# RandomMike1280/AlphaZero-Reversi

Measured on AMD Instinct MI355X. Metric: self-play board-steps/sec @ 800 sims/move, 8x8 Reversi, higher is better.
Workload: dtype u64 rules + f32 NN (fp32 as 2-part f16 split on MFMA)

## Files before the change

### alphazero-reversi_amd/csrc/rvz_play.hip

```cpp
#include <hip/hip_runtime.h>
#include <math.h>
#include <stdint.h>
#include <stdio.h>
#include <stdlib.h>

#include <string>
#include <vector>

#include "../../include/rvz.h"
#include "rvz_engine_host.h"
#include "rvz_h2.hip.h"
#include "rvz_host.hip.h"
#include "rvz_play.hip.h"
#include "rvz_search.hip.h"
#include "rvz_trace.h"

using namespace rvz;


__global__ void k_table_bump(unsigned* gen) {
    if (threadIdx.x == 0) atomicAdd(gen, 1u);
}

int table_bump(rvz_engine* e) {
    if (!e->tgen) return RVZ_OK;
    hipLaunchKernelGGL(k_table_bump, dim3(1), dim3(64), 0, e->stream, e->tgen);
    RVZ_HIP(hipGetLastError(), e);
    return RVZ_OK;
}

void table_free(rvz_engine* e) {
    for (void* p : {(void*)e->tab, (void*)e->tclaim, (void*)e->tgen})
        if (p) (void)hipFree(p);
    e->tab = nullptr;
    e->tclaim = nullptr;
    e->tgen = nullptr;
    e->tslots = 0;
    e->tab_blob = nullptr;
}

extern "C" {

int rvz_play_gate(rvz_engine* e, double fraction, double timeout_us, double late_us) {
    if (!e || !(fraction <= 1.0) || !(timeout_us >= 0.0) || !(late_us >= 0.0) ||
        timeout_us > 1e6 || late_us > 1e6) {
        if (e) e->err = "rvz_play_gate: fraction <= 1 (< 0: the default), 0 <= us <= 1e6";
        return RVZ_EINVAL;
    }
    e->gate_frac = fraction;
    e->gate_us = timeout_us;
    e->gate_late_us = late_us;
    return RVZ_OK;
}

int rvz_play_table(rvz_engine* e, int64_t slots, int32_t max_discs) {
    if (!e) return RVZ_EINVAL;
    if (slots != 0 && (slots < 1024 || (slots & (slots - 1)) != 0 || slots > (1ll << 30) ||
                       max_discs < 4)) {
        e->err = "rvz_play_table: slots a power of two in [1024, 2^30] (or 0), max_discs >= 4";
        return RVZ_EINVAL;
    }
    RVZ_HIP(hipStreamSynchronize(e->stream), e);
    if (slots == e->tslots && slots != 0) {
        e->tmaxd = max_discs;
        return table_bump(e);
    }
    table_free(e);
    if (slots == 0) return RVZ_OK;
    const size_t stride = e->BS == 8 ? TabGeo<8>::STRIDE : TabGeo<6>::STRIDE;
    if (hipMalloc(reinterpret_cast<void**>(&e->tab), (size_t)slots * stride * 8) != hipSuccess ||
        hipMalloc(reinterpret_cast<void**>(&e->tclaim), (size_t)slots * 4) != hipSuccess ||
        hipMalloc(reinterpret_cast<void**>(&e->tgen), 4) != hipSuccess) {
        table_free(e);
        e->err = "hipMalloc failed (rvz_play_table)";
        return RVZ_ENOMEM;
    }
    hipError_t st = hipMemset(e->tab, 0, (size_t)slots * stride * 8);
    if (st == hipSuccess) st = hipMemset(e->tclaim, 0, (size_t)slots * 4);
    if (st == hipSuccess) st = hipMemsetD32(e->tgen, 1u, 1);
    if (st == hipSuccess) st = hipDeviceSynchronize();
    if (st != hipSuccess) {
        table_free(e);
        e->err = std::string("rvz_play_table init: ") + hipGetErrorString(st);
        return RVZ_EHIP;
    }
    e->tslots = slots;
    e->tmaxd = max_discs;
    return RVZ_OK;
}

#ifdef RVZ_WALK_STATS
int rvz_play_walk_read(int32_t n_games, uint64_t* out) {
    const int n = n_games < WALK_STATS_MAX ? n_games : WALK_STATS_MAX;
    std::vector<unsigned long long> a, b;
    if (take_rows(g_wtime, n, a) != RVZ_OK || take_rows(g_ftime, n, b) != RVZ_OK) return RVZ_EHIP;
    for (int i = 0; i < n; ++i) {
        for (int k = 0; k < 5; ++k) out[(size_t)i * 9 + k] = a[(size_t)i * 5 + k];
        for (int k = 0; k < 4; ++k) out[(size_t)i * 9 + 5 + k] = b[(size_t)i * 4 + k];
    }
    return RVZ_OK;
}
#endif

struct PlayScratch {
    int64_t q_next, q_done, gate, queue, x, need, work, logits, value, total;
};
static PlayScratch play_scratch(int64_t G, int NSQ, int NPOL) {
    const auto al4 = [](int64_t n) { return (n + 3) / 4 * 4; };
    int64_t at = 0;
    const auto take = [&](int64_t words) { const int64_t o = at; at += al4(words); return o; };
    PlayScratch s;
    s.q_next = take(4);
    s.q_done = take(2 * al4(G));
    s.gate = take(8 * 32);
    s.queue = at;
    s.x = take(G * 3 * NSQ);
    s.need = take(G);
    s.work = take(G * 192);
    s.logits = take(G * NPOL);
    s.value = take(G);
    s.total = at;
    return s;
}
int64_t rvz_play_scratch_size(const rvz_engine* e) {
    if (!e) return RVZ_EINVAL;
    return play_scratch(e->v.G, e->NSQ, e->NPOL).total;
}

#ifndef RVZ_PLAY_GROUP
#define RVZ_PLAY_GROUP 4
#endif
#ifndef RVZ_PLAY_GATE_FRAC
#define RVZ_PLAY_GATE_FRAC 0.8
#endif
#ifndef RVZ_PLAY_GATE_US
#define RVZ_PLAY_GATE_US 400.0
#endif
#ifndef RVZ_PLAY_GATE_LATE_US
#define RVZ_PLAY_GATE_LATE_US 200.0
#endif
extern "C++" {
template <class T>
static int play_launch(rvz_engine* e, const View& v, const PlayArgs& pa) {
    constexpr int F = T::F, BS = T::BS;
    int cus = 0;
    if (hipDeviceGetAttribute(&cus, hipDeviceAttributeMultiprocessorCount, e->cfg.device) !=
            hipSuccess || cus <= 0)
        cus = 256;
    PlayArgs a = pa;
    const int slots = cus * T::OCC;
    dim3 grid;
    if (a.q_next) {
        if (a.gpw <= 0) a.gpw = RVZ_PLAY_GROUP;
        if (a.gpw > play_gpw_max<F, BS>()) a.gpw = play_gpw_max<F, BS>();
        a.n_groups = (v.G + a.gpw - 1) / a.gpw;
        grid = dim3(a.n_groups < slots ? a.n_groups : slots);
        RVZ_HIP(fill32_async(a.q_next, 0u, (size_t)play_scratch(v.G, e->NSQ, e->NPOL).queue,
                             e->stream), e);
    } else {
        if (a.gpw <= 0) a.gpw = (v.G + slots - 1) / slots;
        if (a.gpw > play_gpw_max<F, BS>()) a.gpw = play_gpw_max<F, BS>();
        a.n_groups = (v.G + a.gpw - 1) / a.gpw;
        grid = dim3(a.n_groups);
    }
    PlayCtx ctx;
    ctx.v = v;
    ctx.a = a;
    hipLaunchKernelGGL((k_play<T::F, T::NB, T::CTW, T::PTW, T::BS, T::OCC>), grid, dim3(256), 0,
                       e->stream, ctx);
    return launch_check(e, "k_play");
}
}

#ifdef RVZ_PLAY_TIMING
int rvz_play_timing_read(uint64_t* host, int n) {
    if (hipMemcpyFromSymbol(host, HIP_SYMBOL(g_play_t), (size_t)n * PLAY_T_SLOTS * 8) != hipSuccess)
        return RVZ_EHIP;
    if (hipMemcpyFromSymbol(host + (size_t)n * PLAY_T_SLOTS, HIP_SYMBOL(g_pass_t),
                            (size_t)n * 6 * 8) != hipSuccess)
        return RVZ_EHIP;
    std::vector<unsigned long long> z((size_t)16384 * PLAY_T_SLOTS, 0ull);
    if (hipMemcpyToSymbol(HIP_SYMBOL(g_pass_t), z.data(), (size_t)16384 * 6 * 8) != hipSuccess)
        return RVZ_EHIP;
    return hipMemcpyToSymbol(HIP_SYMBOL(g_play_t), z.data(), z.size() * 8) == hipSuccess
               ? RVZ_OK : RVZ_EHIP;
}
#endif

struct PlayGate {
    unsigned frac, t, late;
};
static PlayGate play_gate_setting(const rvz_engine* e, bool queue) {
    double frac = e->gate_frac, us = e->gate_us, late = e->gate_late_us;
    if (frac < 0.0) {
        frac = RVZ_PLAY_GATE_FRAC;
        us = RVZ_PLAY_GATE_US;
        late = RVZ_PLAY_GATE_LATE_US;
    }
    if (const char* gs = getenv("RVZ_PLAY_GATE")) {
        double f = 0.0, u = 0.0, l = 0.0;
        const int n = sscanf(gs, "%lf,%lf,%lf", &f, &u, &l);
        frac = n >= 2 ? f : 0.0;
        us = u;
        late = n >= 3 ? l : 0.0;
    }
    PlayGate g;
    g.frac = (queue && frac > 0.0 && us > 0.0) ? (unsigned)(fmin(frac, 1.0) * 65536.0 + 0.5) : 0u;
    g.t = (unsigned)(us * 100.0);
    g.late = late > 0.0 ? (unsigned)(late * 100.0) : 0u;
    return g;
}

int rvz_play(rvz_engine* e, const rvz_play_args* a) {
    const Range trace_range("rvz.play (fused search + h2 evaluator)");
    if (!e || !a) return RVZ_EINVAL;
    if (!a->params || !a->blob || !a->scratch || !a->seeds || !a->plies_done || !a->out_idx ||
        !a->out_p || (a->reset && !a->games_done) || a->plies < 1 || a->blocks < 0 ||
        !h2_tile_ok(e->BS, a->filters) || a->games_per_workgroup < -PLAY_GPW_MAX ||
        e->cfg.leaf_dtype != RVZ_LEAF_F32) {
        e->err = "rvz_play: invalid arguments";
        return RVZ_EINVAL;
    }
    if ((((uintptr_t)a->params | (uintptr_t)a->blob | (uintptr_t)a->scratch) & 15) != 0) {
        e->err = "rvz_play: params, blob and scratch must be 16-byte aligned";
        return RVZ_EINVAL;
    }
    if (in_search(e, "rvz_play")) return RVZ_EINVAL;
    View v = e->v;
    v.live = nullptr;
    v.row_of = nullptr;
    v.live_total = nullptr;
    v.stats = nullptr;
    if ((a->rec_black || a->rec_white || a->rec_side || a->rec_p) &&
        !(a->rec_black && a->rec_white && a->rec_side && a->rec_p)) {
        e->err = "rvz_play: rec_black, rec_white, rec_side and rec_p go together";
        return RVZ_EINVAL;
    }
    PlayArgs pa;
    pa.prm = a->params;
    pa.L = make_layout(a->filters, a->blocks, e->BS);
    pa.blob = a->blob;
    pa.n_blocks = a->blocks;
    pa.ovf = a->ovf;
    const PlayScratch sc = play_scratch(v.G, e->NSQ, e->NPOL);
    const bool queue = a->games_per_workgroup <= 0;
    pa.q_next = queue ? reinterpret_cast<unsigned*>(a->scratch + sc.q_next) : nullptr;
    pa.q_done = queue ? reinterpret_cast<unsigned long long*>(a->scratch + sc.q_done) : nullptr;
    pa.gate = queue ? reinterpret_cast<unsigned long long*>(a->scratch + sc.gate) : nullptr;
    pa.x = a->scratch + sc.x;
    pa.need = reinterpret_cast<int32_t*>(a->scratch + sc.need);
    pa.work = a->scratch + sc.work;
    pa.logits = a->scratch + sc.logits;
    pa.value = a->scratch + sc.value;
    pa.n_groups = 0;
    pa.gpw = queue ? -a->games_per_workgroup : a->games_per_workgroup;
    const PlayGate gate = play_gate_setting(e, queue);
    pa.gate_frac = gate.frac;
    pa.gate_t = gate.t;
    pa.gate_late = gate.late;
    pa.spin_limit = 1u << 26;
    if (const char* sl = getenv("RVZ_PLAY_SPIN_LIMIT")) pa.spin_limit = (unsigned)strtoul(sl, nullptr, 10);
    pa.single_pass = 1;
    if (const char* sp = getenv("RVZ_PLAY_SINGLE_PASS")) pa.single_pass = atoi(sp) != 0;
    pa.S = e->cfg.num_simulations;
    pa.B = e->cfg.batch_size;
    pa.skip_last = a->skip_last_eval && pa.S > pa.B ? 1 : 0;
    pa.skip_forced = a->skip_forced_roots && pa.skip_last ? 1 : 0;
    pa.plies = a->plies;
    pa.budget = a->ply_budget;
    pa.temperature = a->temperature;
    pa.reset = a->reset ? 1 : 0;
    pa.seeds = a->seeds;
    pa.stride = a->seed_stride;
    pa.ply_ctr = a->plies_done;
    pa.done = a->games_done;
    pa.out_idx = a->out_idx;
    pa.out_p = a->out_p;
    pa.hist = a->hist;
    pa.rows = reinterpret_cast<unsigned long long*>(a->rows_evaluated);
    pa.unread = reinterpret_cast<unsigned long long*>(a->rows_unread);
    pa.roots_unread = reinterpret_cast<unsigned long long*>(a->roots_unread);
    pa.tstats = reinterpret_cast<unsigned long long*>(a->table_stats);
    pa.rec_black = a->rec_black;
    pa.rec_white = a->rec_white;
    pa.rec_side = a->rec_side;
    pa.rec_p = a->rec_p;
    pa.tab = nullptr;
    pa.tclaim = nullptr;
    pa.tgen = nullptr;
    pa.tmask = 0;
    pa.tmaxd = 0;
    if (e->tab) {
        if (e->tab_blob != a->blob) {
            if (e->tab_blob) {
                hipStreamCaptureStatus cs = hipStreamCaptureStatusNone;
                if (hipStreamIsCapturing(e->stream, &cs) == hipSuccess &&
                    cs != hipStreamCaptureStatusNone) {
                    e->err = "rvz_play: another weight blob than the table's while the stream is "
                             "capturing (play once eagerly with this evaluator before capturing)";
                    return RVZ_EINVAL;
                }
                const int r = table_bump(e);
                if (r != RVZ_OK) return r;
            }
            e->tab_blob = a->blob;
        }
        pa.tab = e->tab;
        pa.tclaim = e->tclaim;
        pa.tgen = e->tgen;
        pa.tmask = (unsigned)(e->tslots - 1);
        pa.tmaxd = e->tmaxd;
    }
    e->searching = 0;
    int r = RVZ_EINVAL;
    h2_tile(e->BS, a->filters, [&](auto t) { r = play_launch<decltype(t)>(e, v, pa); });
    return r;
}

}
```

### alphazero-reversi_amd/csrc/rvz_play.hip.h

```cpp
#pragma once
#include <hip/hip_runtime.h>
#include <stdint.h>

#include "rvz_h2.hip.h"
#include "rvz_resnet_common.hip.h"
#include "rvz_search.hip.h"

namespace rvz {
namespace {

struct PlayArgs {
    const float* prm;
    Layout L;
    const uint16_t* blob;
    int n_blocks;
    float* x;
    int32_t* need;
    float* work;
    float* logits;
    float* value;
    float* ovf;
    int gpw, plies, skip_last, reset, S, B;
    double temperature;
    int64_t* seeds;
    int64_t stride;
    int64_t* ply_ctr;
    int64_t* done;
    int32_t* out_idx;
    double* out_p;
    int32_t* hist;
    unsigned long long* rows;
    const int32_t* budget;
    unsigned spin_limit;
    int single_pass;
    unsigned long long* tab;
    unsigned* tclaim;
    const unsigned* tgen;
    unsigned tmask;
    int tmaxd;
    unsigned long long* tstats;
    unsigned long long* unread;
    uint64_t* rec_black;
    uint64_t* rec_white;
    int32_t* rec_side;
    double* rec_p;
    unsigned* q_next;
    unsigned long long* q_done;
    int n_groups;
    unsigned long long* gate;
    unsigned gate_frac;
    unsigned gate_t;
    unsigned gate_late;
    int skip_forced;
    unsigned long long* roots_unread;
};
constexpr int PLAY_GPW_MAX = 64;
template <int F, int BS>
__host__ __device__ constexpr bool play_heads_lds() { return F == 64 && BS == 8; }
template <int F, int BS>
__host__ __device__ constexpr int play_gpw_max() {
    return play_heads_lds<F, BS>() ? 8 : PLAY_GPW_MAX;
}
enum : int { PF_QUEUED = 1, PF_READY = 2, PF_DONE = 4, PF_EVAL = 8, PF_HELD = 16 };
constexpr int32_t ERR_SCHED = 16;

template <int BS>
struct TabGeo {
    static constexpr int NSQ = Geo<BS>::NSQ;
    static constexpr int NG = NSQ + 8;
    static constexpr int STRIDE = (NG + 7) / 8 * 8;
};
constexpr int TAB_PROBES = 8;

__device__ __forceinline__ uint64_t tab_mix(uint64_t z) {
    z ^= z >> 30;
    z *= 0xbf58476d1ce4e5b9ull;
    z ^= z >> 27;
    z *= 0x94d049bb133111ebull;
    return z ^ (z >> 31);
}
__device__ __forceinline__ uint64_t tab_hash(uint64_t P, uint64_t O, uint64_t V) {
    return tab_mix(P ^ tab_mix(O ^ tab_mix(V + 0x9e3779b97f4a7c15ull)));
}
template <int NSQ>
__device__ __forceinline__ uint32_t tab_key_word(int idx, uint64_t P, uint64_t O, uint64_t V) {
    const int k = idx - (NSQ + 2);
    const uint64_t w = k < 2 ? P : (k < 4 ? O : V);
    return (k & 1) ? (uint32_t)(w >> 32) : (uint32_t)w;
}

template <int BS>
__device__ __forceinline__ int tab_read(const unsigned long long* __restrict__ tab, uint32_t sl,
                                         uint32_t gen, uint64_t P, uint64_t O, uint64_t V,
                                         int lane, uint64_t& x0, uint64_t& x1) {
    using T = TabGeo<BS>;
    constexpr int NSQ = T::NSQ, NG = T::NG;
    const unsigned long long* e = tab + (size_t)sl * T::STRIDE;
    x0 = 0;
    x1 = 0;
    if (lane < NG) x0 = __hip_atomic_load(e + lane, __ATOMIC_RELAXED, __HIP_MEMORY_SCOPE_AGENT);
    if (NG > 64 && lane < NG - 64)
        x1 = __hip_atomic_load(e + 64 + lane, __ATOMIC_RELAXED, __HIP_MEMORY_SCOPE_AGENT);
    bool stale = false, other = false;
    if (lane < NG) {
        stale |= (uint32_t)(x0 >> 32) != gen;
        if (lane >= NSQ + 2) other |= (uint32_t)x0 != tab_key_word<NSQ>(lane, P, O, V);
    }
    if (NG > 64 && lane < NG - 64) {
        stale |= (uint32_t)(x1 >> 32) != gen;
        if (64 + lane >= NSQ + 2) other |= (uint32_t)x1 != tab_key_word<NSQ>(64 + lane, P, O, V);
    }
    if (__ballot(stale) != 0ull) return 0;
    return __ballot(other) != 0ull ? 1 : 2;
}

template <int BS, int IDX>
__device__ __forceinline__ uint32_t tab_datum(uint64_t x0, uint64_t x1) {
    if constexpr (IDX < 64) return (uint32_t)__builtin_amdgcn_readlane((int)(uint32_t)x0, IDX);
    else return (uint32_t)__builtin_amdgcn_readlane((int)(uint32_t)x1, IDX - 64);
}

template <int BS>
__device__ __forceinline__ bool tab_lookup(const PlayArgs& a, uint32_t gen, uint64_t P,
                                           uint64_t O, uint64_t V, int lane, int g) {
    constexpr int NSQ = Geo<BS>::NSQ, NPOL = Geo<BS>::NPOL;
    const uint64_t h = tab_hash(P, O, V);
    for (int i = 0; i < TAB_PROBES; ++i) {
        const uint32_t sl = (uint32_t)(h + i) & a.tmask;
        uint64_t x0, x1;
        const int r = tab_read<BS>(a.tab, sl, gen, P, O, V, lane, x0, x1);
        if (r == 0) return false;
        if (r == 1) continue;
        float* row = a.logits + (size_t)g * NPOL;
        if (lane < NSQ) row[lane] = __uint_as_float((uint32_t)x0);
        if (lane == 0) {
            row[NSQ] = __uint_as_float(tab_datum<BS, NSQ>(x0, x1));
            a.value[g] = __uint_as_float(tab_datum<BS, NSQ + 1>(x0, x1));
        }
        return true;
    }
    return false;
}

template <int BS>
__device__ __forceinline__ int tab_insert(const PlayArgs& a, uint32_t gen, uint64_t P, uint64_t O,
                                          uint64_t V, int lane, int g) {
    using T = TabGeo<BS>;
    constexpr int NSQ = T::NSQ, NPOL = Geo<BS>::NPOL, NG = T::NG;
    const uint64_t h = tab_hash(P, O, V);
    for (int i = 0; i < TAB_PROBES; ++i) {
        const uint32_t sl = (uint32_t)(h + i) & a.tmask;
        uint32_t c = 0;
        if (lane == 0) c = __hip_atomic_load(a.tclaim + sl, __ATOMIC_RELAXED, __HIP_MEMORY_SCOPE_AGENT);
        c = (uint32_t)__builtin_amdgcn_readfirstlane((int)c);
        if (c == gen) {
            uint64_t x0, x1;
            if (tab_read<BS>(a.tab, sl, gen, P, O, V, lane, x0, x1) == 2) return 0;
            continue;
        }
        uint32_t won = 0;
        if (lane == 0) {
            uint32_t expect = c;
            won = __hip_atomic_compare_exchange_strong(a.tclaim + sl, &expect, gen,
                                                       __ATOMIC_RELAXED, __ATOMIC_RELAXED,
                                                       __HIP_MEMORY_SCOPE_AGENT) ? 1u : 0u;
        }
        if (!__builtin_amdgcn_readfirstlane((int)won)) continue;
        const float* row = a.logits + (size_t)g * NPOL;
        const float val = a.value[g];
        unsigned long long* e = a.tab + (size_t)sl * T::STRIDE;
        const unsigned long long tag = (unsigned long long)gen << 32;
        if (lane < NG) {
            const uint32_t d = lane < NPOL ? __float_as_uint(row[lane])
                               : lane == NSQ + 1 ? __float_as_uint(val)
                                                 : tab_key_word<NSQ>(lane, P, O, V);
            __hip_atomic_store(e + lane, tag | d, __ATOMIC_RELAXED, __HIP_MEMORY_SCOPE_AGENT);
        }
        if (NG > 64 && lane < NG - 64) {
            const int idx = 64 + lane;
            const uint32_t d = idx < NPOL ? __float_as_uint(row[idx])
                               : idx == NSQ + 1 ? __float_as_uint(val)
                                                : tab_key_word<NSQ>(idx, P, O, V);
            __hip_atomic_store(e + idx, tag | d, __ATOMIC_RELAXED, __HIP_MEMORY_SCOPE_AGENT);
        }
        return 1;
    }
    return 0;
}

__device__ __forceinline__ void gate_open(unsigned long long* w, unsigned r) {
    unsigned long long v = __hip_atomic_load(w, __ATOMIC_RELAXED, __HIP_MEMORY_SCOPE_AGENT);
    while ((unsigned)(v >> 32) == r) {
        if (__hip_atomic_compare_exchange_strong(w, &v, (unsigned long long)(r + 1u) << 32,
                                                 __ATOMIC_RELAXED, __ATOMIC_RELAXED,
                                                 __HIP_MEMORY_SCOPE_AGENT)) {
            __hip_atomic_store(w + 1, __builtin_amdgcn_s_memrealtime(), __ATOMIC_RELAXED,
                               __HIP_MEMORY_SCOPE_AGENT);
            return;
        }
    }
}
__device__ __forceinline__ unsigned long long* gate_line(unsigned long long* gate) {
    const unsigned x = (unsigned)__builtin_amdgcn_s_getreg((31 << 11) | 20) & 7u;
    return gate + 16 * x;
}
__device__ __forceinline__ void gate_running(unsigned long long* gate, long long d) {
    __hip_atomic_fetch_add(gate_line(gate) + 2, (unsigned long long)d, __ATOMIC_RELAXED,
                           __HIP_MEMORY_SCOPE_AGENT);
}
__device__ __forceinline__ void play_gate(unsigned long long* gate, unsigned frac, unsigned t,
                                          unsigned late) {
    unsigned long long* w = gate_line(gate);
    if (late) {
        const unsigned long long t_open =
            __hip_atomic_load(w + 1, __ATOMIC_RELAXED, __HIP_MEMORY_SCOPE_AGENT);
        if (t_open && __builtin_amdgcn_s_memrealtime() - t_open < late) return;
    }
    const unsigned long long running =
        __hip_atomic_load(w + 2, __ATOMIC_RELAXED, __HIP_MEMORY_SCOPE_AGENT);
    if (running < 4) return;
    const unsigned k = max(1u, (unsigned)((running * frac) >> 16));
    const unsigned long long old =
        __hip_atomic_fetch_add(w, 1ull, __ATOMIC_RELAXED, __HIP_MEMORY_SCOPE_AGENT);
    const unsigned r = (unsigned)(old >> 32);
    if ((unsigned)old + 1u >= k) {
        gate_open(w, r);
        return;
    }
    const unsigned long long t0 = __builtin_amdgcn_s_memrealtime();
    for (;;) {
        __builtin_amdgcn_s_sleep(2);
        const unsigned long long v = __hip_atomic_load(w, __ATOMIC_RELAXED, __HIP_MEMORY_SCOPE_AGENT);
        if ((unsigned)(v >> 32) != r) return;
        if (__builtin_amdgcn_s_memrealtime() - t0 > t) {
            gate_open(w, r);
            return;
        }
    }
}

struct PlayCtx {
    View v;
    PlayArgs a;
};
__device__ __forceinline__ int opaque_tid() {
    int t = threadIdx.x;
    asm volatile("" : "+v"(t));
    return t;
}
__device__ __forceinline__ const PlayCtx& play_ctx() {
    const __attribute__((address_space(4))) char* p =
        (const __attribute__((address_space(4))) char*)__builtin_amdgcn_kernarg_segment_ptr();
    asm volatile("" : "+s"(p));
    return *(const PlayCtx*)p;
}

#ifdef RVZ_PLAY_TIMING
constexpr int PLAY_T_SLOTS = 14;
__device__ unsigned long long g_play_t[16384][PLAY_T_SLOTS];
#define PT_NOW(t) const unsigned long long t = __builtin_amdgcn_s_memtime()
#define PT_ADD(i, v) if (tid == 0 && blockIdx.x < 16384) g_play_t[blockIdx.x][i] += (v)
#else
#define PT_NOW(t)
#define PT_ADD(i, v)
#endif

template <int F, int NBOARD, int CTW, int PTW, int BS, int OCC>
__global__ __launch_bounds__(256) __attribute__((amdgpu_waves_per_eu(OCC, OCC)))
void k_play(PlayCtx ctx0) {
    (void)ctx0;
    using WT = WaveTilesH<F, CTW, PTW>;
    constexpr bool ILV = RVZ_H2_ILV && NBOARD == 2 && BS == 8 && PTW == 4 && WT::CG == 2;
    using GH = GeoH<NBOARD, BS, 64 * CTW * H2_TM / F, ILV>;
    using C = CfgH<F, GH::NPIX>;
    constexpr int NPOL = Geo<BS>::NPOL;
    constexpr bool HLDS = play_heads_lds<F, BS>();
    constexpr int GMAX = play_gpw_max<F, BS>();
    constexpr bool PLAY_SINGLE = F == 64 && NBOARD == 2 && BS == 8 && (PTW & 1) == 0 && HLDS;
    constexpr int HROW = heads_in_floats(BS) / 16;
    constexpr int SP_BYTES = WPB * (NPOL + 7) * 8;
    static_assert(heads_in_floats(BS) * 4 <= C::RMAX, "heads rows fit");
    static_assert(SP_BYTES + WPB * 624 * 4 <= C::RMAX, "act / reset scratch fits");
    __shared__ __attribute__((aligned(16))) char smem[C::BYTES];
    __shared__ int st_k[GMAX];
    __shared__ int st_f[GMAX];
    __shared__ int st_p[GMAX];
    __shared__ uint64_t st_bits[GMAX * 3];
    __shared__ uint64_t q_bits[(GMAX + NBOARD) * 3];
    __shared__ __attribute__((aligned(16))) float hin[HLDS ? GMAX * HROW : 4];
    __shared__ int q_rows[GMAX + 16];
    __shared__ int s_nq;
    __shared__ float vpart[4][16];
    __shared__ int s_task[2];
    __shared__ unsigned s_tgen;
    const int tid = threadIdx.x;
    const int wave = __builtin_amdgcn_readfirstlane(tid >> 6);
    int E, G, gpw, queue, task_plies;
    {
        const PlayCtx& c = play_ctx();
        E = c.v.E;
        G = c.v.G;
        gpw = c.a.gpw;
        queue = c.a.q_next != nullptr;
        task_plies = queue ? 1 : c.a.plies;
    }
    bool ovf = false;
    __shared__ unsigned s_cnt[5];
    if (tid < 5) s_cnt[tid] = 0u;
    if (tid == 0) {
        const PlayArgs& a = play_ctx().a;
        s_tgen = a.tab ? __hip_atomic_load(a.tgen, __ATOMIC_RELAXED, __HIP_MEMORY_SCOPE_AGENT) : 0u;
    }
    double* sp = reinterpret_cast<double*>(smem) + wave * (NPOL + 7);
    uint32_t* key = reinterpret_cast<uint32_t*>(smem + SP_BYTES) + wave * 624;
    if constexpr (F >= 128 && BS == 8) {
        const PlayArgs& a = play_ctx().a;
        if (tid == 0 && a.gate_frac > 0) gate_running(a.gate, 1);
    }
    PT_NOW(t_start);
    for (int task_i = 0;; ++task_i) {
        int gi, ply0;
        if (!queue) {
            if (task_i > 0) break;
            gi = blockIdx.x;
            ply0 = 0;
        } else {
            PT_NOW(t_q0);
            if (wave == 0) {
                const PlayCtx& c = play_ctx();
                const PlayArgs& a = c.a;
                const int n = a.n_groups;
                const unsigned plies = (unsigned)a.plies;
                const int rot = (int)((unsigned long long)blockIdx.x * (unsigned)n / gridDim.x);
                int tg = -1, tp = 0;
                bool stop = __hip_atomic_load(c.v.err, __ATOMIC_RELAXED,
                                              __HIP_MEMORY_SCOPE_AGENT) & ERR_SCHED;
                unsigned spins = 0;
                while (!stop) {
                    unsigned long long best = ~0ull;
                    bool left = false;
                    for (int i = tid; i < n; i += 64) {
                        const unsigned long long w = __hip_atomic_load(
                            a.q_done + i, __ATOMIC_RELAXED, __HIP_MEMORY_SCOPE_AGENT);
                        const unsigned pub = (unsigned)(w >> 32), cl = (unsigned)w;
                        if (cl < plies) {
                            left = true;
                            if (cl == pub) {
                                const int r = i - rot + (i < rot ? n : 0);
                                const unsigned long long key =
                                    ((unsigned long long)pub << 32) | (unsigned)r;
                                best = key < best ? key : best;
                            }
                        }
                    }
#pragma unroll
                    for (int off = 32; off > 0; off >>= 1) {
                        const unsigned long long o = __shfl_xor(best, off, 64);
                        best = o < best ? o : best;
                    }
                    if (best != ~0ull) {
                        const unsigned p = (unsigned)(best >> 32);
                        int g = (int)(unsigned)best + rot;
                        g -= g >= n ? n : 0;
                        int won = 0;
                        if (tid == 0) {
                            unsigned long long want = ((unsigned long long)p << 32) | p;
                            won = __hip_atomic_compare_exchange_strong(
                                a.q_done + g, &want, want + 1ull, __ATOMIC_RELAXED,
                                __ATOMIC_RELAXED, __HIP_MEMORY_SCOPE_AGENT);
                        }
                        if (__builtin_amdgcn_readfirstlane(won)) {
                            tg = g;
                            tp = (int)p;
                            break;
                        }
                        continue;
                    }
                    if (__ballot(left) == 0) break;
                    __builtin_amdgcn_s_sleep(4);
                    ++spins;
                    PT_ADD(11, 1);
                    if (spins > a.spin_limit ||
                        ((spins & 1023u) == 0 &&
                         (__hip_atomic_load(c.v.err, __ATOMIC_RELAXED,
                                            __HIP_MEMORY_SCOPE_AGENT) & ERR_SCHED))) {
                        if (tid == 0) atomicOr(c.v.err, ERR_SCHED);
                        stop = true;
                    }
                }
                __builtin_amdgcn_fence(__ATOMIC_ACQUIRE, "agent");
                asm volatile("s_waitcnt vmcnt(0)" ::: "memory");
                if (tid == 0) {
                    s_task[0] = tg;
                    s_task[1] = tp;
                }
            }
            __syncthreads();
            gi = __builtin_amdgcn_readfirstlane(s_task[0]);
            ply0 = __builtin_amdgcn_readfirstlane(s_task[1]);
            PT_NOW(t_q1);
            PT_ADD(8, t_q1 - t_q0);
            if (gi < 0) break;
            PT_ADD(9, 1);
        }
        const int g0 = gi * gpw;
        const int ng = min(gpw, G - g0);
        {
            const int32_t* bud = play_ctx().a.budget;
            for (int j = tid; j < ng; j += 256) {
                st_k[j] = 0;
                st_f[j] = (bud && ply0 >= bud[g0 + j]) ? PF_DONE : 0;
                st_p[j] = 0;
            }
        }
        __syncthreads();
        for (;;) {
            PT_NOW(t_c0);
            for (int j = wave; j < ng; j += WPB) {
                const PlayCtx& c = play_ctx();
                const View& v = c.v;
                const PlayArgs& a = c.a;
                const int lane = opaque_tid() & 63;
                const int g = g0 + j;
                int f = __builtin_amdgcn_readfirstlane(st_f[j]);
                if (f & (PF_QUEUED | PF_DONE)) continue;
                int k = __builtin_amdgcn_readfirstlane(st_k[j]);
                int np = __builtin_amdgcn_readfirstlane(st_p[j]);
                WT_NOW(ft_step);
                FT_CNT();
                for (;;) {
                    unsigned long long ab = 0;
                    if (k < E) {
                        const int first = k == 0;
                        const GameS root = load_game(v, g);
                        uint32_t root_meta = 0, carry = LINK_NONE;
                        int root_n = 0;
                        if (!first) {
                            root_meta = v.meta[(size_t)g * v.M];
                            root_n = v.nodes[(size_t)g * v.M].n;
                        } else if (v.memo) {
                            carry = v.carry[g];
                        }
                        if (f & PF_READY) {
                            WT_NOW(ft_e);
                            const ExpIn x = expand_load<BS>(v, g, lane, a.logits, a.value);
                            const int rn =
                                expand_backup_phase<BS>(v, g, lane, x, 1, &root_meta, ab);
                            if (rn >= 0) root_n = rn;
                            f &= ~PF_READY;
                            FT_ADD(0, ft_e);
                        }
                        const int bsz = min(a.B, a.S - k * a.B);
                        const bool unread = a.skip_last && !first && m_nchild(root_meta) >= E - 1;
                        const Forced fz{first && a.skip_forced ? E : 0, a.S, a.B};
                        const int copies = select_phase<BS, float>(v, g, lane, first, bsz, k, root,
                                                                   root_meta, root_n, carry, a.x,
                                                                   a.need, ab, st_bits + 3 * j,
                                                                   unread, fz);
                        if (copies <= -2) {
                            k = E;
                            const int left = -2 - copies;
                            if (lane == 0) {
                                if (left & 255) atomicAdd(&s_cnt[3], (unsigned)(left & 255));
                                if (left >> 8) atomicAdd(&s_cnt[4], 1u);
                            }
                            continue;
                        }
                        ++k;
                        if (copies < 0 && k < E && lane == 0) atomicAdd(&s_cnt[3], 1u);
                        if (copies > 0 && !(k == E && a.skip_last)) {
                            if (a.tab) {
                                const uint64_t P = st_bits[3 * j], O = st_bits[3 * j + 1],
                                               Vb = st_bits[3 * j + 2];
                                WT_NOW(ft_t);
                                const bool hit = __popcll(P | O) <= a.tmaxd &&
                                                 tab_lookup<BS>(a, s_tgen, P, O, Vb, lane, g);
                                WT_ADD(0, ft_t);
                                if (hit) {
                                    __builtin_amdgcn_fence(__ATOMIC_SEQ_CST, "workgroup");
                                    f |= PF_READY;
                                    if (lane == 0) atomicAdd(&s_cnt[1], 1u);
                                    continue;
                                }
                            }
                            f |= PF_QUEUED;
                            break;
                        }
                        continue;
                    }
                    WT_NOW(ft_a);
                    bool over = false;
                    double* outp = a.out_p;
                    if (a.rec_black) {
                        const size_t ri = (size_t)(ply0 + np) * v.G + g;
                        if (lane == 0) {
                            a.rec_black[ri] = v.black[g];
                            a.rec_white[ri] = v.white[g];
                            a.rec_side[ri] = v.status[(size_t)g * 4];
                        }
                        outp = a.rec_p + (size_t)(ply0 + np) * v.G * Geo<BS>::NPOL;
                    }
                    const int idx = act_game<BS>(v, g, lane, sp, (f & PF_READY) ? 1 : 2,
                                                 a.logits, 1, a.value, a.temperature, nullptr, 1,
                                                 a.out_idx, outp, &over);
                    f &= ~PF_READY;
                    int64_t sd = 0;
                    if (lane == 0) {
                        if (idx >= 0) a.ply_ctr[g] += 1;
                        if (a.hist) a.hist[(size_t)(ply0 + np) * v.G + g] = idx;
                        if (a.reset && over) {
                            a.done[g] += 1;
                            sd = a.seeds[g] + a.stride;
                            a.seeds[g] = sd;
                        }
                    }
                    if (a.reset && over) {
                        sd = __shfl(sd, 0);
                        reset_game<BS>(v, g, lane, (uint32_t)(sd & 0xFFFFFFFFll), key);
                    }
                    FT_ADD(1, ft_a);
                    ++np;
                    k = 0;
                    if (np >= task_plies || (a.budget && ply0 + np >= a.budget[g])) {
                        f |= PF_DONE;
                        break;
                    }
                }
                FT_ADD(2, ft_step);
                if (lane == 0) {
                    st_k[j] = k;
                    st_f[j] = f;
                    st_p[j] = np;
                }
            }
            __syncthreads();
            PT_NOW(t_c1);
            PT_ADD(0, t_c1 - t_c0);
            PT_ADD(4, 1);
            if (tid == 0) {
                int n = 0;
                for (int j = 0; j < ng; ++j)
                    if (st_f[j] & PF_QUEUED) ++n;
                int hold = n > NBOARD ? n % NBOARD : 0;
                for (int j = ng - 1; j >= 0; --j) {
                    const int fj = st_f[j];
                    if (!(fj & PF_QUEUED)) continue;
                    if (hold > 0 && !(fj & PF_HELD)) {
                        st_f[j] = fj | PF_HELD;
                        --hold;
                    } else {
                        st_f[j] = (fj & ~PF_HELD) | PF_EVAL;
                    }
                }
                n = 0;
                for (int j = 0; j < ng; ++j)
                    if (st_f[j] & PF_EVAL) {
                        for (int ch = 0; ch < 3; ++ch) q_bits[3 * n + ch] = st_bits[3 * j + ch];
                        q_rows[n++] = g0 + j;
                    }
                for (int i = n; i < n + 16; ++i) q_rows[i] = -1;
                for (int i = 3 * n; i < 3 * (n + NBOARD); ++i) q_bits[i] = 0;
                s_nq = n;
            }
            __syncthreads();
            const int nq = __builtin_amdgcn_readfirstlane(s_nq);
            if (nq == 0) break;
            if (tid == 0) s_cnt[0] += (unsigned)nq;
            PT_NOW(t_c2);

            for (int p0 = 0; p0 < nq; p0 += NBOARD) {
                if constexpr (F >= 128 && BS == 8) {
                    if (play_ctx().a.gate_frac > 0) {
                        if (tid == 0) {
                            const PlayArgs& a = play_ctx().a;
                            play_gate(a.gate, a.gate_frac, a.gate_t, a.gate_late);
                        }
                        __syncthreads();
                    }
                }
                const PlayArgs& a = play_ctx().a;
                PT_NOW(t_p0);
                bool single = false;
                if constexpr (PLAY_SINGLE)
                    single = a.single_pass &&
                             __builtin_amdgcn_readfirstlane(q_rows[p0 + 1]) < 0;
                if (single) {
                    if constexpr (PLAY_SINGLE) {
                        const int t = opaque_tid();
                        ovf |= h2_pass_single<F, CTW, PTW / 2, BS>(
                                   smem, q_bits + 3 * p0, a.prm, a.blob, a.n_blocks, hin, p0, nq,
                                   t, t & 63, __builtin_amdgcn_readfirstlane(t >> 6)) != 0;
                    }
                } else {
                    int gb[NBOARD];
#pragma unroll
                    for (int k = 0; k < NBOARD; ++k) gb[k] = q_rows[p0 + k];
                    const int t = opaque_tid();
                    if constexpr (HLDS)
                        h2_pass<F, NBOARD, CTW, PTW, BS>(
                            smem, a.x, gb, q_bits + 3 * p0, a.prm, a.L, a.blob, a.n_blocks,
                            HeadsInLds<BS>{hin, p0, nq}, t, t & 63,
                            __builtin_amdgcn_readfirstlane(t >> 6), ovf);
                    else
                        h2_pass<F, NBOARD, CTW, PTW, BS>(
                            smem, a.x, gb, q_bits + 3 * p0, a.prm, a.L, a.blob, a.n_blocks,
                            HeadsGlobalIdx<NBOARD>(a.work, gb), t, t & 63,
                            __builtin_amdgcn_readfirstlane(t >> 6), ovf);
                }
                __syncthreads();
#ifdef RVZ_PLAY_TIMING
                if (p0 + NBOARD > nq) {
                    PT_NOW(t_p1);
                    PT_ADD(12, 1);
                    PT_ADD(13, t_p1 - t_p0);
                }
#endif
            }
            PT_NOW(t_c3);
            PT_ADD(1, t_c3 - t_c2);
            PT_ADD(5, (nq + NBOARD - 1) / NBOARD);
            PT_ADD(6, nq);
            for (int h0 = 0; h0 < nq; h0 += 16) {
                const PlayArgs& a = play_ctx().a;
                if constexpr (HLDS)
                    heads_fc16<BS, HeadRowsList, false, false, GMAX>(
                        a.work, HeadRowsList{q_rows + h0}, a.prm, a.L, a.logits, a.value, hin,
                        vpart, opaque_tid());
                else
                    heads_fc16<BS, HeadRowsList, false, true>(
                        a.work, HeadRowsList{q_rows + h0}, a.prm, a.L, a.logits, a.value,
                        reinterpret_cast<float*>(smem), vpart, opaque_tid());
            }
            if (play_ctx().a.tab) {
                __syncthreads();
                for (int i = wave; i < nq; i += WPB) {
                    const PlayArgs& a = play_ctx().a;
                    const uint64_t P = q_bits[3 * i], O = q_bits[3 * i + 1], Vb = q_bits[3 * i + 2];
                    if (__popcll(P | O) <= a.tmaxd)
                        if (tab_insert<BS>(a, s_tgen, P, O, Vb, opaque_tid() & 63, q_rows[i]) &&
                            (opaque_tid() & 63) == 0)
                            atomicAdd(&s_cnt[2], 1u);
                }
            }
            for (int j = tid; j < ng; j += 256)
                if (st_f[j] & PF_EVAL) st_f[j] = (st_f[j] & ~(PF_QUEUED | PF_EVAL)) | PF_READY;
            __syncthreads();
            PT_NOW(t_c4);
            PT_ADD(2, t_c4 - t_c3);
        }
        if (queue) {
            asm volatile("s_waitcnt vmcnt(0)" ::: "memory");
            __syncthreads();
            if (tid == 0) {
                __builtin_amdgcn_fence(__ATOMIC_RELEASE, "agent");
                asm volatile("s_waitcnt vmcnt(0)" ::: "memory");
                __hip_atomic_fetch_add(play_ctx().a.q_done + gi, 1ull << 32, __ATOMIC_RELAXED,
                                       __HIP_MEMORY_SCOPE_AGENT);
                if (ply0 + 1 == play_ctx().a.plies)
                    __hip_atomic_fetch_add(play_ctx().a.q_next, 1u, __ATOMIC_RELAXED,
                                           __HIP_MEMORY_SCOPE_AGENT);
            }
        }
    }
    if constexpr (F >= 128 && BS == 8) {
        const PlayArgs& a = play_ctx().a;
        if (tid == 0 && a.gate_frac > 0) gate_running(a.gate, -1);
    }
#ifdef RVZ_PLAY_TIMING
    {
        PT_NOW(t_end);
        PT_ADD(3, t_end - t_start);
        if (tid == 0 && blockIdx.x < 16384)
            g_play_t[blockIdx.x][10] = __builtin_amdgcn_s_memrealtime();
        if (tid == 0 && blockIdx.x < 16384)
            g_play_t[blockIdx.x][7] =
                ((unsigned long long)__builtin_amdgcn_s_getreg((31 << 11) | 20) << 32) |
                __builtin_amdgcn_s_getreg((31 << 11) | 4);
    }
#endif
    if (queue && tid == 0) {
        const PlayCtx& c = play_ctx();
        const PlayArgs& a = c.a;
        unsigned spins = 0;
        bool stop = __hip_atomic_load(c.v.err, __ATOMIC_RELAXED, __HIP_MEMORY_SCOPE_AGENT) &
                    ERR_SCHED;
        while (!stop && (int)__hip_atomic_load(a.q_next, __ATOMIC_RELAXED,
                                               __HIP_MEMORY_SCOPE_AGENT) < a.n_groups) {
            __builtin_amdgcn_s_sleep(4);
            ++spins;
            if (spins > a.spin_limit ||
                ((spins & 1023u) == 0 &&
                 (__hip_atomic_load(c.v.err, __ATOMIC_RELAXED, __HIP_MEMORY_SCOPE_AGENT) &
                  ERR_SCHED))) {
                atomicOr(c.v.err, ERR_SCHED);
                stop = true;
            }
        }
    }
    float* ovw = play_ctx().a.ovf;
    if (ovf && ovw) *ovw = 1.0f;
    unsigned long long* rows = play_ctx().a.rows;
    __syncthreads();
    if (rows && tid == 0) atomicAdd(rows, (unsigned long long)s_cnt[0]);
    unsigned long long* ts = play_ctx().a.tstats;
    if (ts && tid == 0) {
        if (s_cnt[1]) atomicAdd(ts, (unsigned long long)s_cnt[1]);
        if (s_cnt[2]) atomicAdd(ts + 1, (unsigned long long)s_cnt[2]);
    }
    unsigned long long* un = play_ctx().a.unread;
    if (un && tid == 0 && s_cnt[3]) atomicAdd(un, (unsigned long long)s_cnt[3]);
    unsigned long long* ur = play_ctx().a.roots_unread;
    if (ur && tid == 0 && s_cnt[4]) atomicAdd(ur, (unsigned long long)s_cnt[4]);
}

}
}
```

Before: 1.830 million.

## Split queued game groups into half-units for finer-grained work stealing

In the persistent queue scheduler, each game group's ply task can now be claimed as two half-units, each covering half the games, with per-half 16-bit claim and publish counters packed into the q_done word. A workgroup claims both halves together when no other workgroups are idle-waiting, tracked by a new waiting counter in q_next[1]. Otherwise it claims one half, so idle workgroups can pick up the other. The aim is to cut tail idling and load imbalance when there are fewer ready groups than workgroups. The cost is more atomic traffic, smaller batches per workgroup when split, and a limit of 65535 plies.

```diff
diff --git a/alphazero-reversi_amd/csrc/rvz_play.hip b/alphazero-reversi_amd/csrc/rvz_play.hip
--- a/alphazero-reversi_amd/csrc/rvz_play.hip
+++ b/alphazero-reversi_amd/csrc/rvz_play.hip
@@ -130,6 +130,9 @@
 #ifndef RVZ_PLAY_GROUP
 #define RVZ_PLAY_GROUP 4
 #endif
+#ifndef RVZ_PLAY_SPLIT
+#define RVZ_PLAY_SPLIT 1
+#endif
 #ifndef RVZ_PLAY_GATE_FRAC
 #define RVZ_PLAY_GATE_FRAC 0.8
 #endif
@@ -154,13 +157,28 @@
         if (a.gpw <= 0) a.gpw = RVZ_PLAY_GROUP;
         if (a.gpw > play_gpw_max<F, BS>()) a.gpw = play_gpw_max<F, BS>();
         a.n_groups = (v.G + a.gpw - 1) / a.gpw;
-        grid = dim3(a.n_groups < slots ? a.n_groups : slots);
+        a.n_units = a.n_groups;
+        if (a.gpw < 2 || a.plies > 0xFFFF) a.split = 0;
+        if (a.split) {
+            a.half = (a.gpw + 1) / 2;
+            const char* rd = getenv("RVZ_PLAY_SPLIT_ROUND");
+            if (rd && atoi(rd) != 0) a.half = (a.half + T::NB - 1) / T::NB * T::NB;
+            if (a.half >= a.gpw) {
+                a.split = 0;
+            } else {
+                const int last = v.G - (a.n_groups - 1) * a.gpw;
+                a.n_units = 2 * (a.n_groups - 1) + (last > a.half ? 2 : 1);
+            }
+        }
+        grid = dim3(a.n_units < slots ? a.n_units : slots);
         RVZ_HIP(fill32_async(a.q_next, 0u, (size_t)play_scratch(v.G, e->NSQ, e->NPOL).queue,
                              e->stream), e);
     } else {
         if (a.gpw <= 0) a.gpw = (v.G + slots - 1) / slots;
         if (a.gpw > play_gpw_max<F, BS>()) a.gpw = play_gpw_max<F, BS>();
         a.n_groups = (v.G + a.gpw - 1) / a.gpw;
+        a.n_units = a.n_groups;
+        a.split = 0;
         grid = dim3(a.n_groups);
     }
     PlayCtx ctx;
@@ -262,6 +280,11 @@
     if (const char* sl = getenv("RVZ_PLAY_SPIN_LIMIT")) pa.spin_limit = (unsigned)strtoul(sl, nullptr, 10);
     pa.single_pass = 1;
     if (const char* sp = getenv("RVZ_PLAY_SINGLE_PASS")) pa.single_pass = atoi(sp) != 0;
+    pa.split = RVZ_PLAY_SPLIT;
+    if (const char* ss = getenv("RVZ_PLAY_SPLIT")) pa.split = atoi(ss);
+    if (pa.split < 0 || pa.split > 2) pa.split = 0;
+    pa.half = 0;
+    pa.n_units = 0;
     pa.S = e->cfg.num_simulations;
     pa.B = e->cfg.batch_size;
     pa.skip_last = a->skip_last_eval && pa.S > pa.B ? 1 : 0;
diff --git a/alphazero-reversi_amd/csrc/rvz_play.hip.h b/alphazero-reversi_amd/csrc/rvz_play.hip.h
--- a/alphazero-reversi_amd/csrc/rvz_play.hip.h
+++ b/alphazero-reversi_amd/csrc/rvz_play.hip.h
@@ -47,6 +47,7 @@
     unsigned* q_next;
     unsigned long long* q_done;
     int n_groups;
+    int split, half, n_units;
     unsigned long long* gate;
     unsigned gate_frac;
     unsigned gate_t;
@@ -256,7 +257,7 @@
 }
 
 #ifdef RVZ_PLAY_TIMING
-constexpr int PLAY_T_SLOTS = 14;
+constexpr int PLAY_T_SLOTS = 15;
 __device__ unsigned long long g_play_t[16384][PLAY_T_SLOTS];
 #define PT_NOW(t) const unsigned long long t = __builtin_amdgcn_s_memtime()
 #define PT_ADD(i, v) if (tid == 0 && blockIdx.x < 16384) g_play_t[blockIdx.x][i] += (v)
@@ -291,7 +292,7 @@
     __shared__ int q_rows[GMAX + 16];
     __shared__ int s_nq;
     __shared__ float vpart[4][16];
-    __shared__ int s_task[2];
+    __shared__ int s_task[3];
     __shared__ unsigned s_tgen;
     const int tid = threadIdx.x;
     const int wave = __builtin_amdgcn_readfirstlane(tid >> 6);
@@ -332,7 +333,10 @@
                 const int n = a.n_groups;
                 const unsigned plies = (unsigned)a.plies;
                 const int rot = (int)((unsigned long long)blockIdx.x * (unsigned)n / gridDim.x);
-                int tg = -1, tp = 0;
+                int tg = -1, tp = 0, tw = 3;
+                const int split = a.split;
+                const int gpw_ = a.gpw, half = a.half, G_ = c.v.G;
+                bool waiting = false;
                 bool stop = __hip_atomic_load(c.v.err, __ATOMIC_RELAXED,
                                               __HIP_MEMORY_SCOPE_AGENT) & ERR_SCHED;
                 unsigned spins = 0;
@@ -342,6 +346,21 @@
                     for (int i = tid; i < n; i += 64) {
                         const unsigned long long w = __hip_atomic_load(
                             a.q_done + i, __ATOMIC_RELAXED, __HIP_MEMORY_SCOPE_AGENT);
+                        if (split) {
+                            const int r = i - rot + (i < rot ? n : 0);
+                            const int nu = min(gpw_, G_ - i * gpw_) > half ? 2 : 1;
+                            for (int u = 0; u < nu; ++u) {
+                                const unsigned cl = (unsigned)(w >> (32 * u)) & 0xFFFFu;
+                                const unsigned pub = (unsigned)(w >> (32 * u + 16)) & 0xFFFFu;
+                                if (cl >= plies) continue;
+                                left = true;
+                                if (cl != pub) continue;
+                                const unsigned long long key =
+                                    ((unsigned long long)pub << 32) | (unsigned)(2 * r + u);
+                                best = key < best ? key : best;
+                            }
+                            continue;
+                        }
                         const unsigned pub = (unsigned)(w >> 32), cl = (unsigned)w;
                         if (cl < plies) {
                             left = true;
@@ -360,9 +379,41 @@
                     }
                     if (best != ~0ull) {
                         const unsigned p = (unsigned)(best >> 32);
-                        int g = (int)(unsigned)best + rot;
+                        int g = (int)((unsigned)best >> (split ? 1 : 0)) + rot;
                         g -= g >= n ? n : 0;
                         int won = 0;
+                        if (split) {
+                            const int u = (int)((unsigned)best & 1u);
+                            if (tid == 0) {
+                                const bool pair =
+                                    split == 1 && !waiting &&
+                                    min(gpw_, G_ - g * gpw_) > half &&
+                                    __hip_atomic_load(a.q_next + 1, __ATOMIC_RELAXED,
+                                                      __HIP_MEMORY_SCOPE_AGENT) == 0u;
+                                const unsigned both = p | (p << 16);
+                                unsigned long long w = __hip_atomic_load(
+                                    a.q_done + g, __ATOMIC_RELAXED, __HIP_MEMORY_SCOPE_AGENT);
+                                while ((unsigned)(w >> (32 * u)) == both) {
+                                    const bool sib = pair && (unsigned)(w >> (32 * (1 - u))) == both;
+                                    const unsigned long long inc =
+                                        sib ? (1ull | (1ull << 32)) : (1ull << (32 * u));
+                                    if (__hip_atomic_compare_exchange_strong(
+                                            a.q_done + g, &w, w + inc, __ATOMIC_RELAXED,
+                                            __ATOMIC_RELAXED, __HIP_MEMORY_SCOPE_AGENT)) {
+                                        won = sib ? 3 : 1 + u;
+                                        break;
+                                    }
+                                }
+                            }
+                            won = __builtin_amdgcn_readfirstlane(won);
+                            if (won) {
+                                tg = g;
+                                tp = (int)p;
+                                tw = won;
+                                break;
+                            }
+                            continue;
+                        }
                         if (tid == 0) {
                             unsigned long long want = ((unsigned long long)p << 32) | p;
                             won = __hip_atomic_compare_exchange_strong(
@@ -377,6 +428,12 @@
                         continue;
                     }
                     if (__ballot(left) == 0) break;
+                    if (split && !waiting) {
+                        waiting = true;
+                        if (tid == 0)
+                            __hip_atomic_fetch_add(a.q_next + 1, 1u, __ATOMIC_RELAXED,
+                                                   __HIP_MEMORY_SCOPE_AGENT);
+                    }
                     __builtin_amdgcn_s_sleep(4);
                     ++spins;
                     PT_ADD(11, 1);
@@ -388,11 +445,15 @@
                         stop = true;
                     }
                 }
+                if (waiting && tid == 0)
+                    __hip_atomic_fetch_sub(a.q_next + 1, 1u, __ATOMIC_RELAXED,
+                                           __HIP_MEMORY_SCOPE_AGENT);
                 __builtin_amdgcn_fence(__ATOMIC_ACQUIRE, "agent");
                 asm volatile("s_waitcnt vmcnt(0)" ::: "memory");
                 if (tid == 0) {
                     s_task[0] = tg;
                     s_task[1] = tp;
+                    s_task[2] = tw;
                 }
             }
             __syncthreads();
@@ -403,8 +464,20 @@
             if (gi < 0) break;
             PT_ADD(9, 1);
         }
-        const int g0 = gi * gpw;
-        const int ng = min(gpw, G - g0);
+        int g0 = gi * gpw;
+        int ng = min(gpw, G - g0);
+        if (const int which = queue ? __builtin_amdgcn_readfirstlane(s_task[2]) : 3; which != 3) {
+            const int half = play_ctx().a.half;
+#ifdef RVZ_PLAY_TIMING
+            if (ng > half) { PT_ADD(14, 1); }
+#endif
+            if (which == 2) {
+                g0 += half;
+                ng -= half;
+            } else {
+                ng = min(ng, half);
+            }
+        }
         {
             const int32_t* bud = play_ctx().a.budget;
             for (int j = tid; j < ng; j += 256) {
@@ -654,11 +727,17 @@
             if (tid == 0) {
                 __builtin_amdgcn_fence(__ATOMIC_RELEASE, "agent");
                 asm volatile("s_waitcnt vmcnt(0)" ::: "memory");
-                __hip_atomic_fetch_add(play_ctx().a.q_done + gi, 1ull << 32, __ATOMIC_RELAXED,
+                const int which = s_task[2];
+                const unsigned long long inc =
+                    !play_ctx().a.split ? 1ull << 32
+                                        : ((which & 1) ? 1ull << 16 : 0ull) |
+                                              ((which & 2) ? 1ull << 48 : 0ull);
+                __hip_atomic_fetch_add(play_ctx().a.q_done + gi, inc, __ATOMIC_RELAXED,
                                        __HIP_MEMORY_SCOPE_AGENT);
                 if (ply0 + 1 == play_ctx().a.plies)
-                    __hip_atomic_fetch_add(play_ctx().a.q_next, 1u, __ATOMIC_RELAXED,
-                                           __HIP_MEMORY_SCOPE_AGENT);
+                    __hip_atomic_fetch_add(play_ctx().a.q_next,
+                                           play_ctx().a.split && which == 3 ? 2u : 1u,
+                                           __ATOMIC_RELAXED, __HIP_MEMORY_SCOPE_AGENT);
             }
         }
     }
@@ -685,7 +764,7 @@
         bool stop = __hip_atomic_load(c.v.err, __ATOMIC_RELAXED, __HIP_MEMORY_SCOPE_AGENT) &
                     ERR_SCHED;
         while (!stop && (int)__hip_atomic_load(a.q_next, __ATOMIC_RELAXED,
-                                               __HIP_MEMORY_SCOPE_AGENT) < a.n_groups) {
+                                               __HIP_MEMORY_SCOPE_AGENT) < a.n_units) {
             __builtin_amdgcn_s_sleep(4);
             ++spins;
             if (spins > a.spin_limit ||
```

After: 1.834 million, median of 6. About the same (+0.2%).
